# SimLeek/pySILEnT

Hardware: AMD Instinct MI355X
Metric: Mpx/s full pyramid line-end pass @1080p, 1/2/4/8 GPU; % HBM roofline (higher is better)
Workload: dtype f32

## Files before the change

### pysilent_amd/csrc/silent_common.h

```cpp
#pragma once

#include <hip/hip_runtime.h>
#include <stdint.h>
#include <string.h>

#include <type_traits>

#include "../../include/silent_hip.h"

namespace silent {

constexpr int kMaxLevels = SILENT_MAX_LEVELS;
constexpr int kWave = 64;

struct LevelTab {
    int n_levels;
    int tiles_per_frame;
    long long frame_px;
    int h[kMaxLevels];
    int w[kMaxLevels];
    int tiles_x[kMaxLevels];
    int tile_start[kMaxLevels + 1];
    long long px_off[kMaxLevels];
};

constexpr int kChunk = 1024;

inline long long fill_level_tab(const silent_extent* levels, int n_levels, int n_frames, int tile_w, int tile_h, const bool* skip, LevelTab* tab) {
    const auto sat = [](long long v) { return (int)(v < 0x7fffffffll ? v : 0x7fffffffll); };
    memset(tab, 0, sizeof(*tab));
    tab->n_levels = n_levels;
    long long px = 0, tiles = 0;
    for (int l = 0; l < n_levels; ++l) {
        const long long h = levels[l].h, w = levels[l].w;
        tab->h[l] = (int)h;
        tab->w[l] = (int)w;
        tab->px_off[l] = px;
        tab->tile_start[l] = sat(tiles);
        const long long tx = tile_h ? (w + tile_w - 1) / tile_w : (h * w + tile_w - 1) / tile_w;
        const long long ty = tile_h ? (h + tile_h - 1) / tile_h : 1;
        tab->tiles_x[l] = (int)tx;
        if (!(skip && skip[l])) tiles += tx * ty;
        px += h * w;
    }
    tab->tile_start[n_levels] = sat(tiles);
    tab->tiles_per_frame = sat(tiles);
    tab->frame_px = px;
    return tiles * (long long)n_frames;
}

struct TileCoord {
    int frame, level, ty, tx;
};

__device__ __forceinline__ unsigned xcd_swizzle(unsigned bid, unsigned n) {
    constexpr unsigned kXcd = 8;
    const unsigned per = n / kXcd, rem = n % kXcd;
    const unsigned x = bid % kXcd, k = bid / kXcd;
    return x * per + (x < rem ? x : rem) + k;
}

__device__ __forceinline__ TileCoord locate_tile(const LevelTab& tab, unsigned bid) {
    TileCoord t;
    t.frame = (int)(bid / (unsigned)tab.tiles_per_frame);
    int rem = (int)(bid - (unsigned)t.frame * (unsigned)tab.tiles_per_frame);
    int l = 0;
#pragma unroll
    for (int i = 1; i < kMaxLevels; ++i)
        if (i < tab.n_levels && rem >= tab.tile_start[i]) l = i;
    t.level = l;
    rem -= tab.tile_start[l];
    t.ty = rem / tab.tiles_x[l];
    t.tx = rem - t.ty * tab.tiles_x[l];
    return t;
}

__device__ __forceinline__ float from_lane_below(float v) {
    return __int_as_float(__builtin_amdgcn_update_dpp(0, __float_as_int(v), 0x138 , 0xf, 0xf, true));
}
__device__ __forceinline__ float from_lane_above(float v) {
    return __int_as_float(__builtin_amdgcn_update_dpp(0, __float_as_int(v), 0x130 , 0xf, 0xf, true));
}

template <typename T>
using global_ptr = __attribute__((address_space(1))) T*;
template <typename T>
__device__ __forceinline__ void advance_rows(global_ptr<T>& p, long long elements) {
    p += elements;
    asm("" : "+s"(p));
}

template <bool F64>
using acc_t = typename std::conditional<F64, double, float>::type;
__device__ __forceinline__ double bpermute_f64(int addr, double v) {
    return __hiloint2double(__builtin_amdgcn_ds_bpermute(addr, __double2hiint(v)), __builtin_amdgcn_ds_bpermute(addr, __double2loint(v)));
}

constexpr int kMirrorNearMin = 5;
__device__ __forceinline__ int mirror_near(int i, int n) {
    i = i < 0 ? -i : i;
    i = i >= n ? 2 * (n - 1) - i : i;
    return min(max(i, 0), n - 1);
}

template <bool EDGE = true>
__device__ __forceinline__ float unit_taps6(float c0, float edge, const float (&w)[6]) {
    const float l1 = from_lane_below(c0), l2 = from_lane_below(l1);
    float r1;
    if constexpr (EDGE)
        r1 = __int_as_float(__builtin_amdgcn_update_dpp(__float_as_int(edge), __float_as_int(c0), 0x130 , 0xf, 0xf, false));
    else
        r1 = from_lane_above(c0);
    const float r2 = from_lane_above(r1), r3 = from_lane_above(r2);
    float h = w[0] * l2;
    h = __builtin_fmaf(w[1], l1, h);
    h = __builtin_fmaf(w[2], c0, h);
    h = __builtin_fmaf(w[3], r1, h);
    h = __builtin_fmaf(w[4], r2, h);
    return __builtin_fmaf(w[5], r3, h);
}
template <bool EDGE = true>
__device__ __forceinline__ double unit_taps6(float c0, float edge, const double (&w)[6]) {
    const float l1 = from_lane_below(c0), l2 = from_lane_below(l1);
    float r1;
    if constexpr (EDGE)
        r1 = __int_as_float(__builtin_amdgcn_update_dpp(__float_as_int(edge), __float_as_int(c0), 0x130 , 0xf, 0xf, false));
    else
        r1 = from_lane_above(c0);
    const float r2 = from_lane_above(r1), r3 = from_lane_above(r2);
    double h = w[0] * (double)l2;
    h = __builtin_fma(w[1], (double)l1, h);
    h = __builtin_fma(w[2], (double)c0, h);
    h = __builtin_fma(w[3], (double)r1, h);
    h = __builtin_fma(w[4], (double)r2, h);
    return __builtin_fma(w[5], (double)r3, h);
}
template <typename FT>
constexpr bool kFrameBytes = std::is_same<FT, unsigned char>::value;
struct FrameRgb8 {
    unsigned char b[3];
    __device__ __forceinline__ explicit operator float() const {
        unsigned short lo;
        __builtin_memcpy(&lo, b, 2);
        return __fmul_rn((float)((int)(lo & 0xffu) + (int)(lo >> 8) + (int)b[2]), 1.0f / 3.0f);
    }
};
static_assert(sizeof(FrameRgb8) == 3 && alignof(FrameRgb8) == 1, "one interleaved uint8 colour pixel");
template <typename FT>
constexpr bool kFrameRgb8 = std::is_same<FT, FrameRgb8>::value;
template <typename FT>
constexpr bool kFrameWords = std::is_same<FT, unsigned short>::value;
template <typename PX>
struct FrameStrided {
    const unsigned char* data;
    long long pixel_stride, row_stride, frame_stride;
};
template <typename FT>
constexpr bool kFrameStrided = false;
template <typename PX>
constexpr bool kFrameStrided<FrameStrided<PX>> = true;
template <typename FT>
constexpr bool kFrame16 = kFrameWords<FT> || std::is_same<FT, FrameStrided<unsigned short>>::value;
template <typename PX>
struct StridedSrc {
    const unsigned char* p;
    long long pixel_stride, row_stride;
    __device__ __forceinline__ float at(long long y, long long x) const {
        return (float)*reinterpret_cast<const PX*>(p + y * row_stride + x * pixel_stride);
    }
};
template <typename FT>
struct FrameKind {
    typedef const FT* __restrict__ param;
    typedef const FT* __restrict__ src;
};
template <typename PX>
struct FrameKind<FrameStrided<PX>> {
    typedef FrameStrided<PX> param;
    typedef StridedSrc<PX> src;
    typedef PX px;
};
template <typename FT>
using frame_param = typename FrameKind<FT>::param;
template <typename FT>
using frame_src = typename FrameKind<FT>::src;
template <typename PX>
__device__ __forceinline__ StridedSrc<PX> frame_of(const FrameStrided<PX>& frames, int frame) {
    return StridedSrc<PX>{frames.data + (long long)frame * frames.frame_stride, frames.pixel_stride, frames.row_stride};
}

struct FrameStridedRgb {
    const unsigned char* data;
    long long pixel_stride, row_stride, frame_stride;
};
template <typename FT>
constexpr bool kFrameRgbView = std::is_same<FT, FrameStridedRgb>::value;
__host__ __device__ __forceinline__ long long rgb_view_col(long long i, long long pixel_stride) {
    const long long p = i / 3;
    return p * pixel_stride + (i - 3 * p);
}
struct StridedRgbSrc {
    const unsigned char* p;
    long long pixel_stride, row_stride;
    __device__ __forceinline__ float at(long long y, long long x, int ch) const { return (float)p[y * row_stride + x * pixel_stride + ch]; }
    __device__ __forceinline__ float atf(long long y, long long i) const { return (float)p[y * row_stride + rgb_view_col(i, pixel_stride)]; }
};
template <>
struct FrameKind<FrameStridedRgb> {
    typedef FrameStridedRgb param;
    typedef StridedRgbSrc src;
};
__device__ __forceinline__ StridedRgbSrc frame_of(const FrameStridedRgb& frames, int frame) {
    return StridedRgbSrc{frames.data + (long long)frame * frames.frame_stride, frames.pixel_stride, frames.row_stride};
}

struct FrameNv12 {
    const unsigned char* y;
    const unsigned char* uv;
    long long y_row_stride, y_frame_stride, uv_row_stride, uv_frame_stride;
    float m[9];
    float oy;
};
template <typename FT>
constexpr bool kFrameNv12 = std::is_same<FT, FrameNv12>::value;
struct FrameP010 {
    const unsigned short* y;
    const unsigned short* uv;
    long long y_row_stride, y_frame_stride, uv_row_stride, uv_frame_stride;
    float m[9];
    float oy, oc;
    int shift;
};
template <typename FT>
constexpr bool kFrameP010 = std::is_same<FT, FrameP010>::value;
struct FrameYuv {
    const unsigned char* y;
    const unsigned char* u;
    const unsigned char* v;
    long long y_pixel_stride, y_row_stride, y_frame_stride;
    long long c_pixel_stride, c_row_stride, c_frame_stride;
    int sx, sy;
    float m[9];
    float oy;
};
template <typename FT>
constexpr bool kFrameYuv = std::is_same<FT, FrameYuv>::value;
struct FrameYuv16 {
    const unsigned short* y;
    const unsigned short* u;
    const unsigned short* v;
    long long y_pixel_stride, y_row_stride, y_frame_stride;
    long long c_pixel_stride, c_row_stride, c_frame_stride;
    int sx, sy;
    float m[9];
    float oy, oc;
    int shift;
    unsigned mask;
};
template <typename FT>
constexpr bool kFrameYuv16 = std::is_same<FT, FrameYuv16>::value;
template <typename FT>
constexpr bool kFrameYuvPair = kFrameNv12<FT> || kFrameP010<FT>;
template <typename FT>
constexpr bool kFrameYuvTriple = kFrameYuv<FT> || kFrameYuv16<FT>;
template <typename FT>
constexpr bool kFrameYuvWide = kFrameP010<FT> || kFrameYuv16<FT>;
template <typename FT>
constexpr bool kFrameYuvFamily = kFrameYuvPair<FT> || kFrameYuvTriple<FT>;
template <typename FT>
constexpr bool kFrameRgbSrc = kFrameRgbView<FT> || kFrameYuvFamily<FT>;
__device__ __forceinline__ float nv12_channel(float yv, float uv, float vv, float m0, float m1, float m2) {
    return fminf(fmaxf(__fadd_rn(__fadd_rn(__fmul_rn(yv, m0), __fmul_rn(uv, m1)), __fmul_rn(vv, m2)), 0.0f), 255.0f);
}
__host__ __device__ __forceinline__ long long nv12_y_col(long long x) { return x; }
__host__ __device__ __forceinline__ long long nv12_uv_col(long long x) { return (x >> 1) * 2; }
template <class D>
struct YuvSrcOps {
    __device__ __forceinline__ float at(long long yy, long long x, int ch) const {
        const D& d = *static_cast<const D*>(this);
        float yv, uvv, vv;
        d.yuv(yy, x, yv, uvv, vv);
        const float a0 = d.m[0], a1 = d.m[1], a2 = d.m[2], b0 = d.m[3], b1 = d.m[4], b2 = d.m[5], c0 = d.m[6], c1 = d.m[7], c2 = d.m[8];
        return nv12_channel(yv, uvv, vv, ch == 0 ? a0 : (ch == 1 ? b0 : c0), ch == 0 ? a1 : (ch == 1 ? b1 : c1), ch == 0 ? a2 : (ch == 1 ? b2 : c2));
    }
    __device__ __forceinline__ float atf(long long yy, long long i) const {
        const long long p = i / 3;
        return at(yy, p, (int)(i - 3 * p));
    }
};
struct Nv12Src : YuvSrcOps<Nv12Src> {
    const unsigned char* y;
    const unsigned char* uv;
    long long y_row_stride, uv_row_stride;
    float m[9];
    float oy;
    __device__ __forceinline__ void yuv(long long yy, long long x, float& yv, float& uvv, float& vv) const {
        const unsigned char* c = uv + (yy >> 1) * uv_row_stride + nv12_uv_col(x);
        unsigned short pair;
        __builtin_memcpy(&pair, c, 2);
        yv = __fsub_rn((float)y[yy * y_row_stride + nv12_y_col(x)], oy);
        uvv = (float)((int)(pair & 0xffu) - 128);
        vv = (float)((int)(pair >> 8) - 128);
    }
};
template <>
struct FrameKind<FrameNv12> {
    typedef FrameNv12 param;
    typedef Nv12Src src;
};

__device__ __forceinline__ void p010_values(unsigned e, unsigned pair, float oy, float oc, int shift, float& yv, float& uv, float& vv) {
    yv = __fsub_rn((float)((e & 0xffffu) >> shift), oy);
    uv = __fsub_rn((float)((pair & 0xffffu) >> shift), oc);
    vv = __fsub_rn((float)((pair >> 16) >> shift), oc);
}
__host__ __device__ __forceinline__ long long p010_y_col(long long x) { return 2 * x; }
__host__ __device__ __forceinline__ long long p010_uv_col(long long x) { return (x >> 1) * 4; }
struct P010Src : YuvSrcOps<P010Src> {
    const unsigned char* y;
    const unsigned char* uv;
    long long y_row_stride, uv_row_stride;
    float m[9];
    float oy, oc;
    int shift;
    __device__ __forceinline__ void yuv(long long yy, long long x, float& yv, float& uvv, float& vv) const {
        unsigned short e;
        unsigned pair;
        __builtin_memcpy(&e, y + yy * y_row_stride + p010_y_col(x), 2);
        __builtin_memcpy(&pair, uv + (yy >> 1) * uv_row_stride + p010_uv_col(x), 4);
        p010_values(e, pair, oy, oc, shift, yv, uvv, vv);
    }
};
template <>
struct FrameKind<FrameP010> {
    typedef FrameP010 param;
    typedef P010Src src;
};

__host__ __device__ __forceinline__ long long yuv_y_col(long long x, long long y_pixel_stride) { return x * y_pixel_stride; }
__host__ __device__ __forceinline__ long long yuv_c_col(long long x, int sx, long long c_pixel_stride) { return (x >> sx) * c_pixel_stride; }
struct YuvSrc : YuvSrcOps<YuvSrc> {
    const unsigned char* y;
    const unsigned char* u;
    const unsigned char* v;
    long long y_pixel_stride, y_row_stride, c_pixel_stride, c_row_stride;
    int sx, sy;
    float m[9];
    float oy;
    __device__ __forceinline__ void yuv(long long yy, long long x, float& yv, float& uvv, float& vv) const {
        const long long c = (yy >> sy) * c_row_stride + yuv_c_col(x, sx, c_pixel_stride);
        yv = __fsub_rn((float)y[yy * y_row_stride + yuv_y_col(x, y_pixel_stride)], oy);
        uvv = (float)((int)u[c] - 128);
        vv = (float)((int)v[c] - 128);
    }
};
template <>
struct FrameKind<FrameYuv> {
    typedef FrameYuv param;
    typedef YuvSrc src;
};

__device__ __forceinline__ void yuv16_values(unsigned ey, unsigned eu, unsigned ev, float oy, float oc, int shift, unsigned mask, float& yv,
                                             float& uv, float& vv) {
    yv = __fsub_rn((float)(((ey & 0xffffu) >> shift) & mask), oy);
    uv = __fsub_rn((float)(((eu & 0xffffu) >> shift) & mask), oc);
    vv = __fsub_rn((float)(((ev & 0xffffu) >> shift) & mask), oc);
}
struct Yuv16Src : YuvSrcOps<Yuv16Src> {
    const unsigned char* y;
    const unsigned char* u;
    const unsigned char* v;
    long long y_pixel_stride, y_row_stride, c_pixel_stride, c_row_stride;
    int sx, sy;
    float m[9];
    float oy, oc;
    int shift;
    unsigned mask;
    __device__ __forceinline__ void yuv(long long yy, long long x, float& yv, float& uvv, float& vv) const {
        const long long c = (yy >> sy) * c_row_stride + yuv_c_col(x, sx, c_pixel_stride);
        unsigned short ey, eu, ev;
        __builtin_memcpy(&ey, y + yy * y_row_stride + yuv_y_col(x, y_pixel_stride), 2);
        __builtin_memcpy(&eu, u + c, 2);
        __builtin_memcpy(&ev, v + c, 2);
        yuv16_values(ey, eu, ev, oy, oc, shift, mask, yv, uvv, vv);
    }
};
template <>
struct FrameKind<FrameYuv16> {
    typedef FrameYuv16 param;
    typedef Yuv16Src src;
};
template <typename FT, typename std::enable_if<kFrameYuvFamily<FT>, int>::type = 0>
__device__ __forceinline__ frame_src<FT> frame_of(const FT& f, int frame) {
    frame_src<FT> s;
    s.y = reinterpret_cast<const unsigned char*>(f.y) + (long long)frame * f.y_frame_stride;
    s.y_row_stride = f.y_row_stride;
    if constexpr (kFrameYuvPair<FT>) {
        s.uv = reinterpret_cast<const unsigned char*>(f.uv) + (long long)frame * f.uv_frame_stride;
        s.uv_row_stride = f.uv_row_stride;
    } else {
        s.u = reinterpret_cast<const unsigned char*>(f.u) + (long long)frame * f.c_frame_stride;
        s.v = reinterpret_cast<const unsigned char*>(f.v) + (long long)frame * f.c_frame_stride;
        s.y_pixel_stride = f.y_pixel_stride;
        s.c_pixel_stride = f.c_pixel_stride;
        s.c_row_stride = f.c_row_stride;
        s.sx = f.sx;
        s.sy = f.sy;
    }
#pragma unroll
    for (int i = 0; i < 9; ++i) s.m[i] = f.m[i];
    s.oy = f.oy;
    if constexpr (kFrameYuvWide<FT>) {
        s.oc = f.oc;
        s.shift = f.shift;
    }
    if constexpr (kFrameYuv16<FT>) s.mask = f.mask;
    return s;
}

template <typename FT>
constexpr bool kFrameNarrow = kFrameBytes<FT> || kFrameRgb8<FT> || kFrameWords<FT> || kFrameStrided<FT>;
template <typename FT>
constexpr bool kFrameType = std::is_same<FT, float>::value || kFrameNarrow<FT> || kFrameRgbView<FT> || kFrameYuvFamily<FT>;
template <typename FT>
constexpr size_t frame_px_bytes(int plan_channels) { return kFrameRgb8<FT> ? 3 : kFrameWords<FT> ? 2 : kFrameBytes<FT> ? 1 : 4 * (size_t)plan_channels; }
template <typename FT>
constexpr const char* kFrameSuffix =
    kFrameStrided<FT> ? (kFrame16<FT> ? "_view16" : "_view") : kFrameRgb8<FT> ? "_u8x3" : kFrameWords<FT> ? "_u16" : kFrameBytes<FT> ? "_u8" : "";

template <typename FT = float>
__device__ __forceinline__ float unit_edge_column(const FT* __restrict__ src, long long row_stride, int col, int src_w, int src_x0,
                                                  int y_first, int n_rows, int src_h, int src_y0, int lane, int px_stride = 1) {
    const long long sx = (long long)(mirror_near(col, src_w) + src_x0) * px_stride;
    return (float)src[(long long)(mirror_near(y_first + min(lane, n_rows - 1), src_h) + src_y0) * row_stride + sx];
}
template <typename PX>
__device__ __forceinline__ float unit_edge_column(const StridedSrc<PX>& src, long long, int col, int src_w, int src_x0, int y_first,
                                                  int n_rows, int src_h, int src_y0, int lane, int = 1) {
// ... 61 lines not shown
```

### pysilent_amd/csrc/silent_gray.h

```cpp
#pragma once

#include "silent_common.h"

namespace silent {

struct GrayW {
    float cs[9];
    float end[9 * 8];
};

constexpr int kGrayCols = 60;
constexpr int kGrayTW = 4 * kGrayCols;
constexpr int kGrayTH = 16;

template <bool NT = false>
__device__ __forceinline__ void store_row_k8(float* __restrict__ row_base ,
                                             const float (&acc)[8], float* s_slab ,
                                             int lane, int first, int count) {
    typedef float nf4 __attribute__((ext_vector_type(4)));
    nf4* slab4 = reinterpret_cast<nf4*>(s_slab);
    slab4[lane * 2 + 0] = nf4{acc[0], acc[1], acc[2], acc[3]};
    slab4[lane * 2 + 1] = nf4{acc[4], acc[5], acc[6], acc[7]};
    __builtin_amdgcn_wave_barrier();
    const nf4 a = slab4[lane], b = slab4[64 + lane];
// ... 298 lines not shown

#ifndef SILENT_FUSED_COLS
#define SILENT_FUSED_COLS 56
#endif
constexpr int kFusedCols = SILENT_FUSED_COLS;
static_assert(kFusedCols >= 16 && kFusedCols <= 56 && kFusedCols % 4 == 0, "64 lanes = output columns + 4 halo lanes per side");
#ifndef SILENT_FUSED_WAVES
#define SILENT_FUSED_WAVES 4
#endif
constexpr int kFusedWaves = SILENT_FUSED_WAVES;
constexpr int kFusedTW = kFusedWaves * kFusedCols;
#ifndef SILENT_FUSED_TH
#define SILENT_FUSED_TH 16
#endif
constexpr int kFusedTH = SILENT_FUSED_TH;

struct FusedLevel {
    int src_y0, src_x0, src_h, src_w;
    int zoom_h, zoom_w, out_h, out_w;
    int tiles_x, tile_start;
    long long px_off;
};

struct FusedTab {
    int n, tiles_per_frame, H, W;
    long long frame_px;
    float wx[6], wy[6];
    FusedLevel lv[kMaxLevels];
};
struct FusedTab64 : FusedTab {
    double w64[6];
};
template <bool F64>
using FusedTabT = typename std::conditional<F64, FusedTab64, FusedTab>::type;

template <int K, int R, bool KP = false, bool F64 = false, typename ST = float, typename FT = float>
__global__ __launch_bounds__(64 * kFusedWaves) void gray_unit_fused_kernel(frame_param<FT> frames,
                                                              float* __restrict__ pyr, ST* __restrict__ cs_out,
                                                              ST* __restrict__ end_out, const FusedTabT<F64> tab,
                                                              const GrayW wts, float clip_hi, const GrayKp kp = GrayKp{}) {
    static_assert(!kStoreHalf<ST> || (!KP && !F64), "float16 storage: no keypoint epilogue, no float64 accumulation");
    static_assert(kFrameType<FT> && (!kFrameNarrow<FT> || !F64), "uint8 / uint16 frames: float32 accumulation only");
    __shared__ __attribute__((aligned(16))) float s_slab[K == 8 && !kStoreHalf<ST> ? kFusedWaves * 512 : 4];
    const unsigned bid = blockIdx.x;
    const int frame = (int)(bid / (unsigned)tab.tiles_per_frame);
    int rem = (int)(bid - (unsigned)frame * (unsigned)tab.tiles_per_frame);
    int li = 0;
#pragma unroll
    for (int i = 1; i < kMaxLevels; ++i)
        if (i < tab.n && rem >= tab.lv[i].tile_start) li = i;
    const FusedLevel& lv = tab.lv[li];
    rem -= lv.tile_start;
    const int ty = rem / lv.tiles_x, tx = rem - ty * lv.tiles_x;

    const int lane = threadIdx.x & 63;
    const int wave = __builtin_amdgcn_readfirstlane(threadIdx.x >> 6);
    const int xw0 = tx * kFusedTW + wave * kFusedCols;
    if (xw0 >= lv.out_w) return;
    const int y0 = ty * R;
    const int ox = xw0 + lane - 4;
    const int W = tab.W;
    frame_src<FT> src;
    if constexpr (kFrameStrided<FT>) src = frame_of(frames, frame);
    else src = frames + (long long)frame * tab.H * W;
    const long long base_px = (long long)frame * tab.frame_px + lv.px_off;

    const long long sx = mirror_near(ox, lv.src_w) + lv.src_x0;
    float in[R + 9];
#pragma unroll
    for (int i = 0; i < R + 9; ++i)
    {
        if constexpr (kFrameStrided<FT>) in[i] = src.at(mirror_near(y0 - 4 + i, lv.src_h) + lv.src_y0, sx);
        else in[i] = (float)src[(long long)(mirror_near(y0 - 4 + i, lv.src_h) + lv.src_y0) * W + sx];
    }
    float xcol = unit_edge_column(src, W, xw0 + 60, lv.src_w, lv.src_x0, y0 - 4, R + 9, lv.src_h, lv.src_y0, lane);
#pragma unroll
    for (int i = 0; i < R + 9; ++i) asm volatile("" ::"v"(in[i]));
    asm volatile("" : "+v"(xcol));

    const bool col_in = ox >= 0 && ox < lv.out_w;
    const bool out_lane = lane >= 4 && lane < 4 + kFusedCols && ox < lv.out_w;
    GrayKpAcc ka;
    acc_t<F64> hw[6] = {0, 0, 0, 0, 0, 0};
    float iw[3][3], cw[3][3];
#pragma unroll
    for (int a = 0; a < 3; ++a)
#pragma unroll
        for (int b = 0; b < 3; ++b) iw[a][b] = cw[a][b] = 0.0f;

#pragma unroll
    for (int i = 0; i < R + 9; ++i) {
        {
            acc_t<F64> h;
            if constexpr (F64) h = unit_taps6(in[i], unit_edge(xcol, i), tab.w64);
            else h = unit_taps6(in[i], unit_edge(xcol, i), tab.wx);
#pragma unroll
            for (int j = 0; j < 5; ++j) hw[j] = hw[j + 1];
            hw[5] = h;
        }
        if (i >= 5) {
            const int p = y0 + i - 7;
            float v;
            if constexpr (F64) {
                v = unit_vsum_f64(tab.w64, hw);
            } else {
                v = tab.wy[0] * hw[0];
#pragma unroll
                for (int j = 1; j < 6; ++j) v = __builtin_fmaf(tab.wy[j], hw[j], v);
            }
            v = (p < lv.zoom_h && ox < lv.zoom_w) ? v : 0.0f;
            if (p >= y0 && p < y0 + R && p < lv.out_h && out_lane) pyr[base_px + (long long)p * lv.out_w + ox] = v;
            v = (p >= 0 && p < lv.out_h && col_in) ? v : 0.0f;
#pragma unroll
            for (int b = 0; b < 3; ++b) {
                iw[0][b] = iw[1][b];
                iw[1][b] = iw[2][b];
            }
            iw[2][1] = v;
            iw[2][0] = from_lane_below(v);
            iw[2][2] = from_lane_above(v);
        }
        if (i >= 7) {
            const int c = y0 + i - 8;
            float acc = 0.0f;
            if constexpr (F64) {
                acc = gray_cs_f64(iw, wts.cs);
            } else {
#pragma unroll
                for (int dy = 0; dy < 3; ++dy)
#pragma unroll
                    for (int dx = 0; dx < 3; ++dx) acc = __builtin_fmaf(iw[dy][dx], wts.cs[dy * 3 + dx], acc);
            }
            float cs = relu_tf(acc);
            cs = (c >= 0 && c < lv.out_h && col_in) ? cs : 0.0f;
#pragma unroll
            for (int b = 0; b < 3; ++b) {
                cw[0][b] = cw[1][b];
                cw[1][b] = cw[2][b];
            }
            cw[2][1] = cs;
            cw[2][0] = from_lane_below(cs);
            cw[2][2] = from_lane_above(cs);
        }
        if (i >= 9) {
            const int y = y0 + i - 9;
            if (y < lv.out_h) {
                const long long px = base_px + (long long)y * lv.out_w + ox;
                if constexpr (kStoreHalf<ST>) {
                    if (cs_out)
                        store_cs_row<false>(cs_out + (base_px + (long long)y * lv.out_w + (xw0 - 4)), cw[1][1], lane, 4,
                                            min(kFusedCols, lv.out_w - xw0));
                } else if (cs_out && out_lane) cs_out[px] = cw[1][1];
                if (end_out) {
                    float acc[K];
                    if constexpr (F64) {
                        gray_end_f64<K>(cw, wts.end, clip_hi, acc);
                    } else {
#pragma unroll
                        for (int k = 0; k < K; ++k) acc[k] = 0.0f;
#pragma unroll
                        for (int dy = 0; dy < 3; ++dy)
#pragma unroll
                            for (int dx = 0; dx < 3; ++dx)
#pragma unroll
                                for (int k = 0; k < K; ++k)
                                    acc[k] = __builtin_fmaf(cw[dy][dx], wts.end[(dy * 3 + dx) * K + k], acc[k]);
                        relu_clip_tf(acc, clip_hi);
                    }
                    if constexpr (KP) gray_kp_pixel<K>(kp, acc, y, ox, lv.out_h, lv.out_w, out_lane, kp.value_out + px, ka);
                    if constexpr (K == 8) {
                        const int ncols = min(kFusedCols, lv.out_w - xw0);
                        store_row_k8(end_out + (base_px + (long long)y * lv.out_w + (xw0 - 4)) * 8, acc,
                                     s_slab + wave * 512, lane, 4, ncols);
                    } else if (out_lane) {
                        ST* __restrict__ po = end_out + px * K;
                        if constexpr (kStoreHalf<ST>) {
                            store_end_px<K, false>(po, acc);
                        } else if constexpr (K == 4) {
                            *reinterpret_cast<float4*>(po) = make_float4(acc[0], acc[1], acc[2], acc[3]);
                        } else {
#pragma unroll
                            for (int k = 0; k < K; ++k) po[k] = acc[k];
                        }
                    }
                }
            }
            if constexpr (KP) {
                if (kp_group_ends(i - 9, R)) gray_kp_group_end(kp, ka, frame, kp.level[li], ty, (i - 9) / kSumRows, ox, lv.out_w, out_lane);
            }
        }
    }
    if constexpr (KP) gray_kp_tile_end(kp, ka, frame, kp.level[li], lane);
}

constexpr int kStreamSlots = 5;
__host__ __device__ constexpr int stream_slots(int layout, int g) {
    return layout == 0 ? (g == 0 ? 4 : (g == 1 ? 3 : (g <= 3 ? 2 : 1))) : (g == 0 ? 5 : (g == 1 ? 4 : (g == 2 ? 3 : (g <= 4 ? 2 : 1))));
}
constexpr int kStreamRows = kFusedTH + 8;
__host__ __device__ constexpr int stream_pad_levels(int g) { return g <= 4 ? 4 : 7; }
__host__ __device__ constexpr int stream_w_off(int layout, int gp, int g, bool f64 = false) {
    int o = gp;
    for (int h = 0; h < g; ++h) o += stream_slots(layout, h) * (f64 ? 2 : 1);
    return o;
}
__host__ __device__ constexpr int kStreamProgRow(int layout, int gp, bool f64 = false) {
    return (stream_w_off(layout, gp, gp, f64) + 3) / 4 * 4;
}
__host__ __device__ constexpr int stream_rec_ints(bool f64) { return f64 ? 16 : 8; }
__host__ __device__ constexpr int stream_done_shift(int layout) { return layout == 0 ? 4 : 8; }
__host__ __device__ constexpr int stream_row_shift(int layout) { return layout == 0 ? 8 : 12; }

struct StreamTab {
    int G;
    int tiles_y, waves_x;
    const int* row_prog;
    const int* col_hdr;
    const int* col_rec;
    long long px_off[8];
    int out_w[8];
};

struct StreamCol {
    int x0, n, lane4;
    float w[6];
};
__device__ __forceinline__ StreamCol stream_col(const StreamTab& st, int g, int wx_tile, int lane) {
    const int gg = min(g, st.G - 1);
    const int* __restrict__ h = st.col_hdr + ((long long)gg * st.waves_x + wx_tile) * 2;
    const int4* __restrict__ rec = reinterpret_cast<const int4*>(st.col_rec + (((long long)gg * st.waves_x + wx_tile) * 64 + lane) * 8);
    const int4 a = rec[0], b = rec[1];
    StreamCol c;
    c.x0 = h[0];
    c.n = g < st.G ? h[1] : 0;
    c.lane4 = a.x * 4;
    c.w[0] = __int_as_float(a.y);
    c.w[1] = __int_as_float(a.z);
    c.w[2] = __int_as_float(a.w);
    c.w[3] = __int_as_float(b.x);
    c.w[4] = __int_as_float(b.y);
    c.w[5] = __int_as_float(b.z);
    return c;
}
struct StreamCol64 {
    int x0, n, lane4;
    double w[6];
};
__device__ __forceinline__ StreamCol64 stream_col64(const StreamTab& st, int g, int wx_tile, int lane) {
    const int gg = min(g, st.G - 1);
    const int* __restrict__ h = st.col_hdr + ((long long)gg * st.waves_x + wx_tile) * 2;
    const int4* __restrict__ rec = reinterpret_cast<const int4*>(st.col_rec + (((long long)gg * st.waves_x + wx_tile) * 64 + lane) * 16);
    const int4 a = rec[0], b = rec[1], d = rec[2], e = rec[3];
    StreamCol64 c;
    c.x0 = h[0];
    c.n = g < st.G ? h[1] : 0;
    c.lane4 = a.x * 4;
    c.w[0] = __hiloint2double(a.w, a.z);
    c.w[1] = __hiloint2double(b.y, b.x);
    c.w[2] = __hiloint2double(b.w, b.z);
    c.w[3] = __hiloint2double(d.y, d.x);
    c.w[4] = __hiloint2double(d.w, d.z);
    c.w[5] = __hiloint2double(e.y, e.x);
    return c;
}
template <bool F64>
using StreamColT = typename std::conditional<F64, StreamCol64, StreamCol>::type;
template <bool F64>
__device__ __forceinline__ StreamColT<F64> stream_col_t(const StreamTab& st, int g, int wx_tile, int lane) {
    if constexpr (F64) return stream_col64(st, g, wx_tile, lane);
    else return stream_col(st, g, wx_tile, lane);
}
template <int L, int G, int GR, int PR>
__device__ __forceinline__ void stream_level_f64(int g, const int (&cur)[PR], float c0, double (&vacc)[kStreamSlots],
                                                 const StreamCol64 (&col)[GR > 0 ? GR : 1], const StreamTab& st, int wx_tile, int lane,
                                                 float* __restrict__ pyr, long long frame_px0, int C, int ch) {
    const int meta = cur[g];
#pragma unroll
    for (int k = 0; k < stream_slots(L, g); ++k) {
        const int e = stream_w_off(L, G, g, true) + 2 * k;
        const double w = __hiloint2double(cur[e + 1], cur[e]);
        const double prev = (meta >> k) & 1 ? 0.0 : vacc[k];
        vacc[k] = __builtin_fma(w, (double)c0, prev);
    }
    const int done = (meta >> stream_done_shift(L)) & 7;
    if (done != 7) {
        const int oy = meta >> stream_row_shift(L);
        double v = vacc[0];
#pragma unroll
        for (int k = 1; k < stream_slots(L, g); ++k) v = done == k ? vacc[k] : v;
        const StreamCol64 cr = g < GR ? col[g < GR ? g : 0] : stream_col64(st, g, wx_tile, lane);
        double acc = cr.w[0] * bpermute_f64(cr.lane4, v);
#pragma unroll
        for (int t = 1; t < 6; ++t) acc = __builtin_fma(cr.w[t], bpermute_f64(cr.lane4 + 4 * t, v), acc);
        if (lane < cr.n) pyr[(frame_px0 + st.px_off[g] + (long long)oy * st.out_w[g] + cr.x0 + lane) * C + ch] = (float)acc;
    }
}
#ifndef SILENT_STREAM_REG_LEVELS
#define SILENT_STREAM_REG_LEVELS 3
#endif
constexpr int kStreamRegLevels = SILENT_STREAM_REG_LEVELS;

template <int K, int G>
constexpr bool kStreamTwoBodies = K == 4 && G <= 4;

template <bool INTERIOR, int K, int G, int L, bool KP, bool F64, typename ST, typename FT>
__device__ __forceinline__ void gray_stream_tile(frame_param<FT> frames, float* __restrict__ pyr, ST* __restrict__ cs_out,
                                                 ST* __restrict__ end_out, const FusedTabT<F64> tab, const StreamTab st, const GrayW wts,
                                                 float clip_hi, const GrayKp kp, float* s_slab, float (*s_rows)[kStreamRows][64],
                                                 int frame, int ty, int tx, int wave, int lane) {
#include "silent_gray_stream_tile.h"
}

template <int K, int G, int L = 0, bool KP = false, bool F64 = false, typename ST = float, typename FT = float>
__global__ __launch_bounds__(64 * kFusedWaves) void gray_stream_kernel(frame_param<FT> frames, float* __restrict__ pyr,
                                                          ST* __restrict__ cs_out, ST* __restrict__ end_out,
                                                          const FusedTabT<F64> tab, const StreamTab st, const GrayW wts,
                                                          float clip_hi, unsigned opts, const GrayKp kp = GrayKp{}) {
    static_assert(!kStoreHalf<ST> || (!KP && !F64), "float16 storage: no keypoint epilogue, no float64 accumulation");
    static_assert(kFrameType<FT> && (!kFrameNarrow<FT> || !F64), "uint8 / uint16 frames: float32 accumulation only");
    __shared__ __attribute__((aligned(16))) float s_slab[K == 8 && !kStoreHalf<ST> ? kFusedWaves * 512 : 4];
    __shared__ __attribute__((aligned(16))) float s_rows[kFusedWaves][kStreamRows][64];
    const unsigned bid = (opts & 1u) ? xcd_swizzle(blockIdx.x, gridDim.x) : blockIdx.x;
    const int frame = (int)(bid / (unsigned)tab.tiles_per_frame);
    const int rem = (int)(bid - (unsigned)frame * (unsigned)tab.tiles_per_frame);
    const int ty = rem / tab.lv[0].tiles_x, tx = rem - ty * tab.lv[0].tiles_x;
    const int lane = threadIdx.x & 63;
    const int wave = __builtin_amdgcn_readfirstlane(threadIdx.x >> 6);
    if constexpr (kStreamTwoBodies<K, G>) {
        const FusedLevel& u = tab.lv[0];
        const int wy0 = ty * kFusedTH, wx0 = tx * kFusedTW + wave * kFusedCols;
        const int lim_h = min(u.src_h, min(u.zoom_h, u.out_h)), lim_w = min(u.src_w, min(u.zoom_w, u.out_w));
        if (wy0 >= 4 && wy0 + kFusedTH + 4 < lim_h && wx0 >= 4 && wx0 + 60 < lim_w)
            gray_stream_tile<true, K, G, L, KP, F64, ST, FT>(frames, pyr, cs_out, end_out, tab, st, wts, clip_hi, kp, s_slab, s_rows, frame, ty, tx, wave, lane);
        else
            gray_stream_tile<false, K, G, L, KP, F64, ST, FT>(frames, pyr, cs_out, end_out, tab, st, wts, clip_hi, kp, s_slab, s_rows, frame, ty, tx, wave, lane);
    } else {
#include "silent_gray_stream_tile_general.h"
    }
}

template <int C, int G, int L = 0, bool F64 = false, typename FT = float>
__global__ __launch_bounds__(64 * kFusedWaves) void pyramid_stream_kernel(frame_param<FT> frames, float* __restrict__ pyr,
                                                             const FusedTabT<F64> tab, const StreamTab st) {
    static_assert(kFrameType<FT> && (!kFrameNarrow<FT> || (!F64 && C == 1)), "uint8 / uint16 frames: one channel, float32 accumulation");
    constexpr int R = kFusedTH, NR = kStreamRows;
    __shared__ float s_rows[kFusedWaves][NR][64];
    const unsigned bid = blockIdx.x;
    const int frame = (int)(bid / (unsigned)tab.tiles_per_frame);
    const int rem = (int)(bid - (unsigned)frame * (unsigned)tab.tiles_per_frame);
    const FusedLevel& lv = tab.lv[0];
    const int ty = rem / lv.tiles_x, tx = rem - ty * lv.tiles_x;
    const int lane = threadIdx.x & 63;
    const int wave = __builtin_amdgcn_readfirstlane(threadIdx.x >> 6);
    const int xw0 = tx * kFusedTW + wave * kFusedCols;
    if (xw0 >= lv.out_w) return;
    const int wx_tile = tx * kFusedWaves + wave;
    const int y0 = ty * R;
    const int ox = xw0 + lane - 4;
    const long long WC = (long long)tab.W * C;
    frame_src<FT> src;
    if constexpr (kFrameStrided<FT>) src = frame_of(frames, frame);
    else src = frames + (long long)frame * tab.H * WC;
    const long long frame_px0 = (long long)frame * tab.frame_px;
    const long long base_px = frame_px0 + lv.px_off;
    const long long sx = (long long)(mirror_near(ox, lv.src_w) + lv.src_x0) * C;

    constexpr int GR = G < kStreamRegLevels ? G : kStreamRegLevels;
    StreamColT<F64> col[GR > 0 ? GR : 1];
#pragma unroll
    for (int g = 0; g < GR; ++g) col[g] = stream_col_t<F64>(st, g, wx_tile, lane);
    const int eff_h = min(lv.zoom_h, lv.out_h), eff_w = min(lv.zoom_w, lv.out_w);
    const bool col_eff = ox >= 0 && ox < eff_w;
    const bool out_lane = lane >= 4 && lane < 4 + kFusedCols && ox < lv.out_w;
    static_assert(G == stream_pad_levels(G), "row programs are padded to 4 or 7 levels");
    constexpr int PR = kStreamProgRow(L, G, F64);
    typedef const __attribute__((address_space(4))) int* const_int_ptr;
    const_int_ptr prog = (const_int_ptr)(st.row_prog + (long long)ty * (NR * PR));

#pragma unroll 1
    for (int ch = 0; ch < C; ++ch) {
        float in[R + 8];
#pragma unroll
        for (int i = 0; i < R + 8; ++i)
            if constexpr (kFrameStrided<FT>) in[i] = src.at(mirror_near(y0 - 4 + i, lv.src_h) + lv.src_y0, sx);
            else in[i] = (float)src[(long long)(mirror_near(y0 - 4 + i, lv.src_h) + lv.src_y0) * WC + sx + ch];
#pragma unroll
        for (int i = 0; i < R + 8; ++i) asm volatile("" ::"v"(in[i]));
#pragma unroll
        for (int i = 0; i < R + 8; ++i) s_rows[wave][i][lane] = in[i];

        {
            acc_t<F64> vacc[G][kStreamSlots];
#pragma unroll
            for (int g = 0; g < G; ++g)
#pragma unroll
                for (int k = 0; k < kStreamSlots; ++k) vacc[g][k] = 0.0f;
            int cur[PR], nxt[PR];
#pragma unroll
            for (int e = 0; e < PR; ++e) cur[e] = prog[e];
            float c0 = s_rows[wave][0][lane];
#pragma unroll 1
            for (int i = 0; i < NR; ++i) {
                const int inx = min(i + 1, NR - 1);
#pragma unroll
                for (int e = 0; e < PR; ++e) nxt[e] = prog[inx * PR + e];
                const float c_next = s_rows[wave][inx][lane];
#pragma unroll
                for (int g = 0; g < G; ++g) {
                    const int meta = cur[g];
                    if (!(meta & 128)) continue;
                    if constexpr (F64) {
                        stream_level_f64<L, G, GR>(g, cur, c0, vacc[g], col, st, wx_tile, lane, pyr, frame_px0, C, ch);
                    } else {
#pragma unroll
                        for (int k = 0; k < stream_slots(L, g); ++k) {
                            const float w = __int_as_float(cur[stream_w_off(L, G, g) + k]);
                            const float prev = (meta >> k) & 1 ? 0.0f : vacc[g][k];
                            vacc[g][k] = __builtin_fmaf(w, c0, prev);
                        }
                        const int done = (meta >> stream_done_shift(L)) & 7;
                        if (done != 7) {
                            const int oy = meta >> stream_row_shift(L);
                            float v = vacc[g][0];
#pragma unroll
                            for (int k = 1; k < stream_slots(L, g); ++k) v = done == k ? vacc[g][k] : v;
                            const int vbits = __float_as_int(v);
                            const StreamCol cr = g < GR ? col[g < GR ? g : 0] : stream_col(st, g, wx_tile, lane);
                            float acc = cr.w[0] * __int_as_float(__builtin_amdgcn_ds_bpermute(cr.lane4, vbits));
#pragma unroll
                            for (int q = 1; q < 6; ++q)
                                acc = __builtin_fmaf(cr.w[q], __int_as_float(__builtin_amdgcn_ds_bpermute(cr.lane4 + 4 * q, vbits)), acc);
                            if (lane < cr.n)
                                pyr[(frame_px0 + st.px_off[g] + (long long)oy * st.out_w[g] + cr.x0 + lane) * C + ch] = acc;
                        }
                    }
                }
#pragma unroll
                for (int e = 0; e < PR; ++e) cur[e] = nxt[e];
                c0 = c_next;
            }
        }

        acc_t<F64> hw[6] = {0, 0, 0, 0, 0, 0};
#pragma unroll
        for (int i = 0; i < R + 8; ++i) {
            acc_t<F64> h;
            if constexpr (F64) h = unit_taps6<false>(s_rows[wave][i][lane], 0.0f, tab.w64);
            else h = unit_taps6<false>(s_rows[wave][i][lane], 0.0f, tab.wx);
#pragma unroll
            for (int j = 0; j < 5; ++j) hw[j] = hw[j + 1];
            hw[5] = h;
            if (i >= 7 && i < R + 7) {
                const int p = y0 + i - 7;
                float v;
                if constexpr (F64) {
                    v = unit_vsum_f64(tab.w64, hw);
                } else {
                    v = tab.wy[0] * hw[0];
#pragma unroll
                    for (int j = 1; j < 6; ++j) v = __builtin_fmaf(tab.wy[j], hw[j], v);
                }
                v = (p < eff_h && col_eff) ? v : 0.0f;
                if (p < lv.out_h && out_lane) pyr[(base_px + (long long)p * lv.out_w + ox) * C + ch] = v;
            }
        }
    }
}

}
```

### pysilent_amd/csrc/silent_gray_stream_tile.h

```cpp
    constexpr int R = kFusedTH, NR = kStreamRows;
    const FusedLevel& lv = tab.lv[0];
    const int xw0 = tx * kFusedTW + wave * kFusedCols;
    const bool live = xw0 < lv.out_w;
    const int wx_tile = tx * kFusedWaves + wave;
    const int y0 = ty * R;
    const int ox = xw0 + lane - 4;
    const int W = tab.W;
    frame_src<FT> src;
    if constexpr (kFrameStrided<FT>) src = frame_of(frames, frame);
    else src = frames + (long long)frame * tab.H * W;
    const long long frame_px0 = (long long)frame * tab.frame_px;
    const long long base_px = frame_px0 + lv.px_off;

    float in[R + 8];
    float in_last = 0.0f, xcol = 0.0f;
    constexpr int GR = G < kStreamRegLevels ? G : kStreamRegLevels;
    StreamColT<F64> col[GR > 0 ? GR : 1];
    if constexpr (INTERIOR) {
        const int sy0 = y0 - 4 + lv.src_y0, sx0 = xw0 - 4 + lv.src_x0;
        if constexpr (kFrameStrided<FT>) {
            auto row = src;
            global_ptr<const unsigned char> rp = (global_ptr<const unsigned char>)(src.p + (sy0 * src.row_stride + sx0 * src.pixel_stride));
#pragma unroll
            for (int i = 0; i < R + 9; ++i) {
                row.p = (const unsigned char*)rp;
                const float f = row.at(0, lane);
                if (i < R + 8) in[i < R + 8 ? i : 0] = f;
                else in_last = f;
                advance_rows(rp, src.row_stride);
            }
            xcol = src.at(sy0 + min(lane, R + 8), sx0 + 64);
        } else {
            global_ptr<const FT> rp = (global_ptr<const FT>)(src + ((long long)sy0 * W + sx0));
#pragma unroll
            for (int i = 0; i < R + 9; ++i) {
                const float f = (float)((const FT*)rp)[lane];
                if (i < R + 8) in[i < R + 8 ? i : 0] = f;
                else in_last = f;
                advance_rows(rp, W);
            }
            xcol = (float)src[(long long)(sy0 + min(lane, R + 8)) * W + (sx0 + 64)];
        }
#pragma unroll
        for (int g = 0; g < GR; ++g) col[g] = stream_col_t<F64>(st, g, wx_tile, lane);
    } else {
        const long long sx = mirror_near(ox, lv.src_w) + lv.src_x0;
#pragma unroll
        for (int i = 0; i < R + 8; ++i) in[i] = 0.0f;
#pragma unroll
        for (int g = 0; g < GR; ++g) {
            col[g].x0 = col[g].n = col[g].lane4 = 0;
#pragma unroll
            for (int j = 0; j < 6; ++j) col[g].w[j] = 0.0f;
        }
        if (live) {
#pragma unroll
            for (int i = 0; i < R + 8; ++i)
            {
                if constexpr (kFrameStrided<FT>) in[i] = src.at(mirror_near(y0 - 4 + i, lv.src_h) + lv.src_y0, sx);
                else in[i] = (float)src[(long long)(mirror_near(y0 - 4 + i, lv.src_h) + lv.src_y0) * W + sx];
            }
            if constexpr (kFrameStrided<FT>) in_last = src.at(mirror_near(y0 + R + 4, lv.src_h) + lv.src_y0, sx);
            else in_last = (float)src[(long long)(mirror_near(y0 + R + 4, lv.src_h) + lv.src_y0) * W + sx];
            xcol = unit_edge_column(src, W, xw0 + 60, lv.src_w, lv.src_x0, y0 - 4, R + 9, lv.src_h, lv.src_y0, lane);
#pragma unroll
            for (int g = 0; g < GR; ++g) col[g] = stream_col_t<F64>(st, g, wx_tile, lane);
        }
        if (!live) return;
    }
#pragma unroll
    for (int i = 0; i < R + 8; ++i) asm volatile("" ::"v"(in[i]));
    asm volatile("" : "+v"(in_last), "+v"(xcol));
#pragma unroll
    for (int g = 0; g < GR; ++g) {
        asm volatile("" ::"v"(col[g].lane4));
#pragma unroll
        for (int j = 0; j < 6; ++j) asm volatile("" ::"v"(col[g].w[j]));
    }
#pragma unroll
    for (int i = 0; i < R + 8; ++i) s_rows[wave][i][lane] = in[i];

    acc_t<F64> vacc[G][kStreamSlots];
#pragma unroll
    for (int g = 0; g < G; ++g)
#pragma unroll
        for (int k = 0; k < kStreamSlots; ++k) vacc[g][k] = 0.0f;
    static_assert(G == stream_pad_levels(G), "row programs are padded to 4 or 7 levels");
    constexpr int PR = kStreamProgRow(L, G, F64);
    typedef const __attribute__((address_space(4))) int* const_int_ptr;
    const_int_ptr prog = (const_int_ptr)(st.row_prog + (long long)ty * (NR * PR));
    static_assert(NR % 2 == 0, "pass 2 runs two stream rows per iteration");
    constexpr int HS = 2;
    int rec[2][PR];
    float cv[2];
#pragma unroll
    for (int e = 0; e < PR; ++e) rec[0][e] = prog[e];
    cv[0] = s_rows[wave][0][lane];
#pragma unroll 1
    for (int i = 0; i < NR; i += HS) {
#pragma unroll
        for (int h = 0; h < HS; ++h) {
            const int (&cur)[PR] = rec[h];
            const float c0 = cv[h];
            const int in = min(i + h + 1, NR - 1);
#pragma unroll
            for (int e = 0; e < PR; ++e) rec[h ^ 1][e] = prog[in * PR + e];
            cv[h ^ 1] = s_rows[wave][in][lane];
#pragma unroll
            for (int g = 0; g < G; ++g) {
                const int meta = cur[g];
                if (!(meta & 128)) continue;
                if constexpr (F64) {
                    stream_level_f64<L, G, GR>(g, cur, c0, vacc[g], col, st, wx_tile, lane, pyr, frame_px0, 1, 0);
                } else {
#pragma unroll
                    for (int k = 0; k < stream_slots(L, g); ++k) {
                        const float w = __int_as_float(cur[stream_w_off(L, G, g) + k]);
                        const float prev = (meta >> k) & 1 ? 0.0f : vacc[g][k];
                        vacc[g][k] = __builtin_fmaf(w, c0, prev);
                    }
                    const int done = (meta >> stream_done_shift(L)) & 7;
                    if (done != 7) {
                        const int oy = meta >> stream_row_shift(L);
                        float v = vacc[g][0];
#pragma unroll
                        for (int k = 1; k < stream_slots(L, g); ++k) v = done == k ? vacc[g][k] : v;
                        const int vbits = __float_as_int(v);
                        const StreamCol cr = g < GR ? col[g < GR ? g : 0] : stream_col(st, g, wx_tile, lane);
                        float acc = cr.w[0] * __int_as_float(__builtin_amdgcn_ds_bpermute(cr.lane4, vbits));
#pragma unroll
                        for (int t = 1; t < 6; ++t)
                            acc = __builtin_fmaf(cr.w[t], __int_as_float(__builtin_amdgcn_ds_bpermute(cr.lane4 + 4 * t, vbits)), acc);
                        if (lane < cr.n) pyr[frame_px0 + st.px_off[g] + (long long)oy * st.out_w[g] + cr.x0 + lane] = acc;
                    }
                }
            }
        }
    }

    constexpr bool VW = K <= 4;
    acc_t<F64> wv[6];
    float csw[9], endw[VW ? 9 * K : 1];
#pragma unroll
    for (int j = 0; j < 6; ++j) {
        if constexpr (F64) wv[j] = tab.w64[j];
        else wv[j] = tab.wx[j];
        if constexpr (VW) asm volatile("" : "+v"(wv[j]));
    }
#pragma unroll
    for (int j = 0; j < 9; ++j) {
        csw[j] = wts.cs[j];
        if constexpr (VW) asm volatile("" : "+v"(csw[j]));
    }
    if constexpr (VW) {
#pragma unroll
        for (int j = 0; j < 9 * K; ++j) {
            endw[j] = wts.end[j];
            asm volatile("" : "+v"(endw[j]));
        }
    }
    const int eff_h = min(lv.zoom_h, lv.out_h), eff_w = min(lv.zoom_w, lv.out_w);
    const bool col_eff = INTERIOR || (ox >= 0 && ox < eff_w);
    const bool col_in = INTERIOR || (ox >= 0 && ox < lv.out_w);
    const bool out_lane = lane >= 4 && lane < 4 + kFusedCols && (INTERIOR || ox < lv.out_w);
    const long long wave_px = base_px + (xw0 - 4);
    global_ptr<float> prow = (global_ptr<float>)(pyr + (wave_px + (long long)y0 * lv.out_w));
    global_ptr<ST> crow = (global_ptr<ST>)(cs_out + (wave_px + (long long)y0 * lv.out_w));
    global_ptr<ST> erow = (global_ptr<ST>)(end_out + (wave_px + (long long)y0 * lv.out_w) * K);
    {
        GrayKpAcc ka;
        acc_t<F64> hw[6] = {0, 0, 0, 0, 0, 0};
        float iw[3][3], cw[3][3];
#pragma unroll
        for (int a = 0; a < 3; ++a)
#pragma unroll
            for (int b = 0; b < 3; ++b) iw[a][b] = cw[a][b] = 0.0f;
#pragma unroll
        for (int i = 0; i < R + 9; ++i) {
            {
                const float c0 = i < R + 8 ? s_rows[wave][i < R + 8 ? i : 0][lane] : in_last;
                const acc_t<F64> h = unit_taps6(c0, unit_edge(xcol, i), wv);
#pragma unroll
                for (int j = 0; j < 5; ++j) hw[j] = hw[j + 1];
                hw[5] = h;
            }
            if (i >= 5) {
                const int p = y0 + i - 7;
                float v;
                if constexpr (F64) {
                    v = unit_vsum_f64(wv, hw);
                } else {
                    v = wv[0] * hw[0];
#pragma unroll
                    for (int j = 1; j < 6; ++j) v = __builtin_fmaf(wv[j], hw[j], v);
                }
                if constexpr (!INTERIOR) v = (p >= 0 && p < eff_h && col_eff) ? v : 0.0f;
                if (p >= y0 && p < y0 + R && (INTERIOR || p < lv.out_h)) {
                    if (out_lane) __builtin_nontemporal_store(v, (float*)prow + lane);
                    advance_rows(prow, lv.out_w);
                }
#pragma unroll
                for (int b = 0; b < 3; ++b) {
                    iw[0][b] = iw[1][b];
                    iw[1][b] = iw[2][b];
                }
                iw[2][1] = v;
                iw[2][0] = from_lane_below(v);
                iw[2][2] = from_lane_above(v);
            }
            if (i >= 7) {
                const int c = y0 + i - 8;
                float acc = 0.0f;
                if constexpr (F64) {
                    acc = gray_cs_f64(iw, csw);
                } else {
#pragma unroll
                    for (int dy = 0; dy < 3; ++dy)
#pragma unroll
                        for (int dx = 0; dx < 3; ++dx) acc = __builtin_fmaf(iw[dy][dx], csw[dy * 3 + dx], acc);
                }
                const float cs = (INTERIOR || (c >= 0 && c < lv.out_h && col_in)) && !(acc < 0.0f) ? acc : 0.0f;
#pragma unroll
                for (int b = 0; b < 3; ++b) {
                    cw[0][b] = cw[1][b];
                    cw[1][b] = cw[2][b];
                }
                cw[2][1] = cs;
                cw[2][0] = from_lane_below(cs);
                cw[2][2] = from_lane_above(cs);
            }
            if (i >= 9) {
                const int y = y0 + i - 9;
                if (INTERIOR || y < lv.out_h) {
                    ST* __restrict__ crow_y = (ST*)crow;
                    ST* __restrict__ erow_y = (ST*)erow;
                    if constexpr (kStoreHalf<ST>) {
                        if (cs_out) store_cs_row<true>(crow_y, cw[1][1], lane, 4, INTERIOR ? kFusedCols : min(kFusedCols, lv.out_w - xw0));
                    } else if (cs_out) {
                        if (out_lane) __builtin_nontemporal_store(cw[1][1], crow_y + lane);
                    }
                    if (end_out) {
                        float acc[K];
                        if constexpr (F64) {
                            gray_end_f64<K>(cw, VW ? endw : wts.end, clip_hi, acc);
                        } else {
#pragma unroll
                            for (int k = 0; k < K; ++k) acc[k] = 0.0f;
#pragma unroll
                            for (int dy = 0; dy < 3; ++dy)
#pragma unroll
                                for (int dx = 0; dx < 3; ++dx)
#pragma unroll
                                    for (int k = 0; k < K; ++k) {
                                        const int wi = (dy * 3 + dx) * K + k;
                                        if constexpr (VW) acc[k] = __builtin_fmaf(cw[dy][dx], endw[wi], acc[k]);
                                        else acc[k] = __builtin_fmaf(cw[dy][dx], wts.end[wi], acc[k]);
                                    }
                            relu_clip_tf(acc, clip_hi);
                        }
                        if constexpr (KP) gray_kp_pixel<K>(kp, acc, y, ox, lv.out_h, lv.out_w, out_lane, kp.value_out + (wave_px + (long long)y * lv.out_w) + lane, ka);
                        if constexpr (K == 8) {
                            const int ncols = INTERIOR ? kFusedCols : min(kFusedCols, lv.out_w - xw0);
                            store_row_k8<true>(erow_y, acc, s_slab + wave * 512, lane, 4, ncols);
                        } else {
                            if (out_lane) store_end_lane<K>(erow_y, lane, acc);
                        }
                    }
                    advance_rows(crow, lv.out_w);
                    advance_rows(erow, (long long)lv.out_w * K);
                }
                if constexpr (KP) {
                    if (kp_group_ends(i - 9, R)) gray_kp_group_end(kp, ka, frame, kp.level[0], ty, (i - 9) / kSumRows, ox, lv.out_w, out_lane);
                }
            }
        }
        if constexpr (KP) gray_kp_tile_end(kp, ka, frame, kp.level[0], lane);
    }
```

Before: 143,100.

## Read horizontal taps from padded per-wave LDS slab instead of DPP lane shifts

The two-body stream tile now stores its input rows, plus the extra edge column, into a padded per-wave LDS slab with a pitch of 65. The six horizontal taps for each row are loaded directly from LDS, prefetched one row ahead, instead of being built with DPP lane shuffles and an edge select. The separate in_last register is folded into the input array. This aims to cut the DPP dependency chain and edge handling in the inner loop, at the cost of more LDS reads and a larger shared allocation that could lower occupancy.

After: 142,500. Within noise of the previous version (-0.4%).

```diff
diff --git a/pysilent_amd/csrc/silent_common.h b/pysilent_amd/csrc/silent_common.h
--- a/pysilent_amd/csrc/silent_common.h
+++ b/pysilent_amd/csrc/silent_common.h
@@ -85,6 +85,8 @@
 template <typename T>
 using global_ptr = __attribute__((address_space(1))) T*;
 template <typename T>
+using lds_ptr = __attribute__((address_space(3))) T*;
+template <typename T>
 __device__ __forceinline__ void advance_rows(global_ptr<T>& p, long long elements) {
     p += elements;
     asm("" : "+s"(p));
@@ -134,6 +136,19 @@
     h = __builtin_fma(w[3], (double)r1, h);
     h = __builtin_fma(w[4], (double)r2, h);
     return __builtin_fma(w[5], (double)r3, h);
+}
+constexpr int kTapPitch = 65, kTapPad = 2;
+__device__ __forceinline__ float unit_taps6_row(const float (&taps)[6], const float (&w)[6]) {
+    float h = w[0] * taps[0];
+#pragma unroll
+    for (int j = 1; j < 6; ++j) h = __builtin_fmaf(w[j], taps[j], h);
+    return h;
+}
+__device__ __forceinline__ double unit_taps6_row(const float (&taps)[6], const double (&w)[6]) {
+    double h = w[0] * (double)taps[0];
+#pragma unroll
+    for (int j = 1; j < 6; ++j) h = __builtin_fma(w[j], (double)taps[j], h);
+    return h;
 }
 template <typename FT>
 constexpr bool kFrameBytes = std::is_same<FT, unsigned char>::value;
diff --git a/pysilent_amd/csrc/silent_gray.h b/pysilent_amd/csrc/silent_gray.h
--- a/pysilent_amd/csrc/silent_gray.h
+++ b/pysilent_amd/csrc/silent_gray.h
@@ -624,11 +624,13 @@
 
 template <int K, int G>
 constexpr bool kStreamTwoBodies = K == 4 && G <= 4;
+constexpr int kStreamTapSlab = kTapPad + (kFusedTH + 9) * kTapPitch + kTapPad;
+static_assert(kFusedWaves * kStreamTapSlab * 4 + 16  <= 160 * 1024 / 6, "six blocks of a two-body stream kernel per CU");
 
 template <bool INTERIOR, int K, int G, int L, bool KP, bool F64, typename ST, typename FT>
 __device__ __forceinline__ void gray_stream_tile(frame_param<FT> frames, float* __restrict__ pyr, ST* __restrict__ cs_out,
                                                  ST* __restrict__ end_out, const FusedTabT<F64> tab, const StreamTab st, const GrayW wts,
-                                                 float clip_hi, const GrayKp kp, float* s_slab, float (*s_rows)[kStreamRows][64],
+                                                 float clip_hi, const GrayKp kp, float* s_slab, lds_ptr<float> s_rows ,
                                                  int frame, int ty, int tx, int wave, int lane) {
 #include "silent_gray_stream_tile.h"
 }
@@ -649,13 +651,15 @@
     const int lane = threadIdx.x & 63;
     const int wave = __builtin_amdgcn_readfirstlane(threadIdx.x >> 6);
     if constexpr (kStreamTwoBodies<K, G>) {
+        __shared__ float s_taps[kFusedWaves][kStreamTapSlab];
+        const lds_ptr<float> s_wave = (lds_ptr<float>)&s_taps[wave][kTapPad];
         const FusedLevel& u = tab.lv[0];
         const int wy0 = ty * kFusedTH, wx0 = tx * kFusedTW + wave * kFusedCols;
         const int lim_h = min(u.src_h, min(u.zoom_h, u.out_h)), lim_w = min(u.src_w, min(u.zoom_w, u.out_w));
         if (wy0 >= 4 && wy0 + kFusedTH + 4 < lim_h && wx0 >= 4 && wx0 + 60 < lim_w)
-            gray_stream_tile<true, K, G, L, KP, F64, ST, FT>(frames, pyr, cs_out, end_out, tab, st, wts, clip_hi, kp, s_slab, s_rows, frame, ty, tx, wave, lane);
+            gray_stream_tile<true, K, G, L, KP, F64, ST, FT>(frames, pyr, cs_out, end_out, tab, st, wts, clip_hi, kp, s_slab, s_wave, frame, ty, tx, wave, lane);
         else
-            gray_stream_tile<false, K, G, L, KP, F64, ST, FT>(frames, pyr, cs_out, end_out, tab, st, wts, clip_hi, kp, s_slab, s_rows, frame, ty, tx, wave, lane);
+            gray_stream_tile<false, K, G, L, KP, F64, ST, FT>(frames, pyr, cs_out, end_out, tab, st, wts, clip_hi, kp, s_slab, s_wave, frame, ty, tx, wave, lane);
     } else {
 #include "silent_gray_stream_tile_general.h"
     }
diff --git a/pysilent_amd/csrc/silent_gray_stream_tile.h b/pysilent_amd/csrc/silent_gray_stream_tile.h
--- a/pysilent_amd/csrc/silent_gray_stream_tile.h
+++ b/pysilent_amd/csrc/silent_gray_stream_tile.h
@@ -12,8 +12,8 @@
     const long long frame_px0 = (long long)frame * tab.frame_px;
     const long long base_px = frame_px0 + lv.px_off;
 
-    float in[R + 8];
-    float in_last = 0.0f, xcol = 0.0f;
+    float in[R + 9];
+    float xcol = 0.0f;
     constexpr int GR = G < kStreamRegLevels ? G : kStreamRegLevels;
     StreamColT<F64> col[GR > 0 ? GR : 1];
     if constexpr (INTERIOR) {
@@ -24,9 +24,7 @@
 #pragma unroll
             for (int i = 0; i < R + 9; ++i) {
                 row.p = (const unsigned char*)rp;
-                const float f = row.at(0, lane);
-                if (i < R + 8) in[i < R + 8 ? i : 0] = f;
-                else in_last = f;
+                in[i] = row.at(0, lane);
                 advance_rows(rp, src.row_stride);
             }
             xcol = src.at(sy0 + min(lane, R + 8), sx0 + 64);
@@ -34,9 +32,7 @@
             global_ptr<const FT> rp = (global_ptr<const FT>)(src + ((long long)sy0 * W + sx0));
 #pragma unroll
             for (int i = 0; i < R + 9; ++i) {
-                const float f = (float)((const FT*)rp)[lane];
-                if (i < R + 8) in[i < R + 8 ? i : 0] = f;
-                else in_last = f;
+                in[i] = (float)((const FT*)rp)[lane];
                 advance_rows(rp, W);
             }
             xcol = (float)src[(long long)(sy0 + min(lane, R + 8)) * W + (sx0 + 64)];
@@ -46,7 +42,7 @@
     } else {
         const long long sx = mirror_near(ox, lv.src_w) + lv.src_x0;
 #pragma unroll
-        for (int i = 0; i < R + 8; ++i) in[i] = 0.0f;
+        for (int i = 0; i < R + 9; ++i) in[i] = 0.0f;
 #pragma unroll
         for (int g = 0; g < GR; ++g) {
             col[g].x0 = col[g].n = col[g].lane4 = 0;
@@ -55,13 +51,11 @@
         }
         if (live) {
 #pragma unroll
-            for (int i = 0; i < R + 8; ++i)
+            for (int i = 0; i < R + 9; ++i)
             {
                 if constexpr (kFrameStrided<FT>) in[i] = src.at(mirror_near(y0 - 4 + i, lv.src_h) + lv.src_y0, sx);
                 else in[i] = (float)src[(long long)(mirror_near(y0 - 4 + i, lv.src_h) + lv.src_y0) * W + sx];
             }
-            if constexpr (kFrameStrided<FT>) in_last = src.at(mirror_near(y0 + R + 4, lv.src_h) + lv.src_y0, sx);
-            else in_last = (float)src[(long long)(mirror_near(y0 + R + 4, lv.src_h) + lv.src_y0) * W + sx];
             xcol = unit_edge_column(src, W, xw0 + 60, lv.src_w, lv.src_x0, y0 - 4, R + 9, lv.src_h, lv.src_y0, lane);
 #pragma unroll
             for (int g = 0; g < GR; ++g) col[g] = stream_col_t<F64>(st, g, wx_tile, lane);
@@ -69,8 +63,8 @@
         if (!live) return;
     }
 #pragma unroll
-    for (int i = 0; i < R + 8; ++i) asm volatile("" ::"v"(in[i]));
-    asm volatile("" : "+v"(in_last), "+v"(xcol));
+    for (int i = 0; i < R + 9; ++i) asm volatile("" ::"v"(in[i]));
+    asm volatile("" : "+v"(xcol));
 #pragma unroll
     for (int g = 0; g < GR; ++g) {
         asm volatile("" ::"v"(col[g].lane4));
@@ -78,7 +72,8 @@
         for (int j = 0; j < 6; ++j) asm volatile("" ::"v"(col[g].w[j]));
     }
 #pragma unroll
-    for (int i = 0; i < R + 8; ++i) s_rows[wave][i][lane] = in[i];
+    for (int i = 0; i < R + 9; ++i) s_rows[i * kTapPitch + lane] = in[i];
+    if (lane < R + 9) s_rows[lane * kTapPitch + 64] = xcol;
 
     acc_t<F64> vacc[G][kStreamSlots];
 #pragma unroll
@@ -95,7 +90,7 @@
     float cv[2];
 #pragma unroll
     for (int e = 0; e < PR; ++e) rec[0][e] = prog[e];
-    cv[0] = s_rows[wave][0][lane];
+    cv[0] = s_rows[lane];
 #pragma unroll 1
     for (int i = 0; i < NR; i += HS) {
 #pragma unroll
@@ -105,7 +100,7 @@
             const int in = min(i + h + 1, NR - 1);
 #pragma unroll
             for (int e = 0; e < PR; ++e) rec[h ^ 1][e] = prog[in * PR + e];
-            cv[h ^ 1] = s_rows[wave][in][lane];
+            cv[h ^ 1] = s_rows[in * kTapPitch + lane];
 #pragma unroll
             for (int g = 0; g < G; ++g) {
                 const int meta = cur[g];
@@ -175,11 +170,18 @@
         for (int a = 0; a < 3; ++a)
 #pragma unroll
             for (int b = 0; b < 3; ++b) iw[a][b] = cw[a][b] = 0.0f;
+        lds_ptr<const float> taps4 = s_rows + (lane - 2);
+        asm("" : "+v"(taps4));
+        float ahead[6];
+#pragma unroll
+        for (int j = 0; j < 6; ++j) ahead[j] = taps4[j];
 #pragma unroll
         for (int i = 0; i < R + 9; ++i) {
             {
-                const float c0 = i < R + 8 ? s_rows[wave][i < R + 8 ? i : 0][lane] : in_last;
-                const acc_t<F64> h = unit_taps6(c0, unit_edge(xcol, i), wv);
+                float taps[6];
+#pragma unroll
+                for (int j = 0; j < 6; ++j) taps[j] = ahead[j];
+                const acc_t<F64> h = unit_taps6_row(taps, wv);
 #pragma unroll
                 for (int j = 0; j < 5; ++j) hw[j] = hw[j + 1];
                 hw[5] = h;
@@ -207,6 +209,14 @@
                 iw[2][1] = v;
                 iw[2][0] = from_lane_below(v);
                 iw[2][2] = from_lane_above(v);
+            }
+            if (i + 1 < R + 9) {
+                if ((i + 1) % 4 == 0) {
+                    taps4 = s_rows + ((i + 1) * kTapPitch + lane - 2);
+                    asm("" : "+v"(taps4));
+                }
+#pragma unroll
+                for (int j = 0; j < 6; ++j) ahead[j] = taps4[((i + 1) % 4) * kTapPitch + j];
             }
             if (i >= 7) {
                 const int c = y0 + i - 8;
```
